# aatifjiwani/lens-flare

Measured on AMD Instinct MI355X. Metric: Mray-surface-intersections/s + frame time, 1080p 256spp double-Gauss, higher is better.
Workload: dtype f32

## Files before the change

### lens-flare_amd/csrc/lf_cull.hip

```cpp
#include <algorithm>
#include <cstdio>
#include <cstdlib>

#include "lf_internal.h"
#include "lf_march_events.h"
#include "lf_march_common.h"

namespace {

using namespace lfm;

constexpr int kWgWaves = 8;
constexpr int kListBits = 12;
constexpr int kListMax = 1 << kListBits;

struct PathTally {
  unsigned long long n_rays = 0, events = 0, n_clip = 0, n_vign = 0, n_tir = 0, n_scene = 0, n_rm_lane = 0, n_rm_rows = 0;
  unsigned long long executed = 0;
  unsigned n_light = 0;
};

template <int VAR>
__device__ __forceinline__ void march_channel_factors(const LfLensDev* __restrict__ lens, float* __restrict__ s_chan, int tid) {
  if (VAR & kVarLights) { lights_channel_factors(lens, s_chan, tid, 64 * kWgWaves); return; }
  if (tid < LF_MAX_LAMBDA * 3) {
    const int l = tid / 3, c = tid - 3 * l;
    s_chan[tid] = l < lens->n_lambda ? lens->sun_radiance[c] * lens->lambda_rgb[l][c] : 0.0f;
  }
}

template <int K, bool W1, int VAR>
__device__ __forceinline__ void march_started_path(const LfLensDev* __restrict__ lens, const LfPairsDev* __restrict__ pairs,
                                                   const int* __restrict__ seq_table, const LfProgRow* __restrict__ rec_table,
                                                   const LfWeightRow* __restrict__ wrec_table, const float* __restrict__ mask,
                                                   const MarchArgs& a, int q, lanemask start_mask, float X, float Y,
                                                   const StartRay& s0, int lane, int acc_slot,
                                                   unsigned long long* __restrict__ s_acc, const float* __restrict__ s_chan,
                                                   PathTally& T) {
  const int n_lambda = lens->n_lambda, prog_recs = pairs->prog_recs;
  const int n_groups = (n_lambda + K - 1) / K;
  const float inv_stop_h = a.inv_stop_h, lobe_thr = a.lobe_thr;
  const float sx = lens->sun_dir[0], sy = lens->sun_dir[1], sz = lens->sun_dir[2];
  const float inv_1mc = lens->sun_inv_one_minus_cos, sun_ss = lens->sun_ss;
  const int n_ev = pairs->ev_cnt[q];
  const int* const seq = seq_table + pairs->ev_off[q];
  for (int g = 0; g < n_groups; g++) {
    const LfProgRow* const recs = rec_table + (size_t)g * (size_t)prog_recs;
    const LfWeightRow* const wrecs = wrec_table + (size_t)g * (size_t)prog_recs;
    Ray r[K];
    lanemask alive[K];
    unsigned nlive = 0u;
#pragma unroll
    for (int j = 0; j < K; j++) {
      r[j] = Ray{X, Y, 0.0f, fmaf(X, X, Y * Y), s0.dx, s0.dy, s0.dz, s0.w0, 1.0f};
      const float ns = lens->n_start[min(g * K + j, n_lambda - 1)];
      r[j].dx *= ns; r[j].dy *= ns; r[j].dz *= ns;
      alive[j] = (g * K + j < n_lambda) ? start_mask : 0ull;
      nlive += (unsigned)__popcll(alive[j]);
    }
    T.n_rays += nlive;
    unsigned ev32 = 0u;
    unsigned se = (unsigned)*(const int __attribute__((address_space(4)))*)(seq);
    int e = 0;
    if (n_ev > 0 && nlive != 0u) for (;;) {
      const unsigned cur = se;
      se = (unsigned)*(const int __attribute__((address_space(4)))*)(seq + e + 1);
      const LfProgRow wr = load_prec(recs, cur & 0xffffu);
      LfWeightRow ww;
      if (W1) ww = load_wrec(wrecs, cur & 0xffffu);
      else { for (int j = 0; j < 3; j++) { ww.fs[j] = 1.0f; ww.fo[j] = 1.0f; ww.fi[j] = 1.0f; } ww.coat = 0; }
      const unsigned kind = cur >> 16;
      lanemask okv[K], gv[K], died = 0ull;
      if (kind & LF_EV_STOP) {
#pragma unroll
        for (int j = 0; j < K; j++) {
          if (K > 1 && __builtin_expect(alive[j] == 0ull, 0)) { okv[j] = 0ull; gv[j] = 0ull; continue; }
          okv[j] = stop_event_var<W1, VAR>(r[j], wr.dzv, wr.h2, inv_stop_h, mask, a.mw, a.mh);
          gv[j] = okv[j];
          died |= alive[j] & ~okv[j];
        }
        if (__builtin_expect(died != 0ull, 0)) {
#pragma unroll
          for (int j = 0; j < K; j++) {
            const unsigned nd = (unsigned)__popcll(alive[j] & ~okv[j]);
            T.n_clip += nd; nlive -= nd; alive[j] &= okv[j];
          }
          if (nlive == 0u) e = n_ev;
        }
      } else {
        if (kind == 0u) {
#pragma unroll
          for (int j = 0; j < K; j++) {
            if (K > 1 && __builtin_expect(alive[j] == 0ull, 0)) { okv[j] = 0ull; gv[j] = 0ull; continue; }
            okv[j] = surface_event<W1>(r[j], wr.dzv, wr.curv, wr.ch, wr.c2, wr.sc, wr.cn22[j], wr.rn2[j],
                                       wr.delta[j], wr.h2, false, false, wr.sgn, gv[j], ww.fs[j], ww.fo[j], ww.fi[j],
                                       CoatSel<VAR>{wrec_table, ww.coat, j});
            died |= alive[j] & ~okv[j];
          }
        } else if (kind == (unsigned)LF_EV_REFLECT) {
#pragma unroll
          for (int j = 0; j < K; j++) {
            if (K > 1 && __builtin_expect(alive[j] == 0ull, 0)) { okv[j] = 0ull; gv[j] = 0ull; continue; }
            okv[j] = surface_event<W1>(r[j], wr.dzv, wr.curv, wr.ch, wr.c2, wr.sc, wr.cn22[j], wr.rn2[j],
                                       wr.delta[j], wr.h2, true, false, wr.sgn, gv[j], ww.fs[j], ww.fo[j], ww.fi[j],
                                       CoatSel<VAR>{wrec_table, ww.coat, j});
            died |= alive[j] & ~okv[j];
          }
        } else {
#pragma unroll
          for (int j = 0; j < K; j++) {
            if (K > 1 && __builtin_expect(alive[j] == 0ull, 0)) { okv[j] = 0ull; gv[j] = 0ull; continue; }
            okv[j] = surface_event<W1>(r[j], wr.dzv, wr.curv, wr.ch, wr.c2, wr.sc, wr.cn22[j], wr.rn2[j],
                                       wr.delta[j], wr.h2, (kind & LF_EV_REFLECT) != 0, (kind & LF_EV_FLAT) != 0,
                                       wr.sgn, gv[j], ww.fs[j], ww.fo[j], ww.fi[j],
                                       CoatSel<VAR>{wrec_table, ww.coat, j});
            died |= alive[j] & ~okv[j];
          }
        }
        if (__builtin_expect(died != 0ull, 0)) {
#pragma unroll
          for (int j = 0; j < K; j++) {
            T.n_vign += (unsigned)__popcll(alive[j] & ~gv[j]);
            T.n_tir += (unsigned)__popcll(alive[j] & gv[j] & ~okv[j]);
            nlive -= (unsigned)__popcll(alive[j] & ~okv[j]);
            alive[j] &= okv[j];
          }
          if (nlive == 0u) e = n_ev;
        }
      }
      ev32 += nlive;
      if (++e >= n_ev) break;
    }
    T.events += ev32;
    T.executed += ev32;
    if (nlive == 0u) continue;
    T.n_scene += nlive;
    lanemask lit[K], lit_any = 0ull;
    if (VAR & kVarLights) {
      lit_any = lights_pretest<K, !W1, VAR>(lens, r, alive, lit);
      if (lit_any == 0ull) continue;
    } else {
#pragma unroll
    for (int j = 0; j < K; j++) {
      const float cg = fmaf(r[j].dx, sx, fmaf(r[j].dy, sy, r[j].dz * sz));
      lit[j] = alive[j] & __ballot(cg > lobe_thr);
      lit_any |= lit[j];
    }
    if (lit_any == 0ull) continue;
    if (!W1) {
      lit_any = lobe_gate<K>(r, lit, sx, sy, sz, sun_ss, inv_1mc);
      if (lit_any == 0ull) continue;
    }
    }
    for (int j = 0; j < K; j++) {
      lanemask lj = lit[0];
#pragma unroll
      for (int jj = 1; jj < K; jj++) lj = (j == jj) ? lit[jj] : lj;
      if (lj == 0ull) continue;
      const int l = g * K + j;
      Ray rw = j == 0 ? r[0] : j == 1 ? r[K > 1 ? 1 : 0] : r[K > 2 ? 2 : 0];
      if (!W1) {
        rw = Ray{X, Y, 0.0f, fmaf(X, X, Y * Y), s0.dx, s0.dy, s0.dz, s0.w0, 1.0f};
        { const float ns = lens->n_start[l]; rw.dx *= ns; rw.dy *= ns; rw.dz *= ns; }
        T.n_rm_lane += (unsigned long long)((unsigned)n_ev * (unsigned)__popcll(lj));
        T.n_rm_rows += (unsigned)n_ev;
        weighted_remarch<VAR>(rw, seq, n_ev, j, recs, wrecs, wrec_table, mask, inv_stop_h, a.mw, a.mh);
      }
      if (VAR & kVarLights) {
        lights_epilogue<VAR>(lens, s_chan, rw, ((lj >> lane) & 1ull) != 0ull, l, &s_acc[acc_slot * 3], T.n_light);
        continue;
      }
      const float qq = lobe_q(rw.dx, rw.dy, rw.dz, sx, sy, sz, sun_ss, inv_1mc);
      const float om = 1.0f - qq;
      float contrib = __fdiv_rn(rw.wn, rw.wd) * (om * om);
      contrib = (((lj >> lane) & 1ull) != 0ull && qq < 1.0f && contrib > 0.0f) ? contrib : 0.0f;
      T.n_light += contrib > 0.0f ? 1u : 0u;
#pragma unroll
      for (int c = 0; c < 3; c++) {
        const float v = contrib * s_chan[l * 3 + c];
        const unsigned long long fx = (unsigned long long)(v * 68719476736.0f);
        if (fx) atomicAdd(&s_acc[acc_slot * 3 + c], fx);
      }
    }
  }
}

template <int K, bool REFLECT, bool FLAT>
__device__ __forceinline__ lanemask surface_rows(Ray (&r)[K], const lanemask (&alive)[K], const LfProgRow& wr, lanemask (&okv)[K],
                                                 lanemask (&gv)[K]) {
  lanemask died = 0ull;
#pragma unroll
  for (int j = 0; j < K; j++) {
    if (K > 1 && __builtin_expect(alive[j] == 0ull, 0)) { okv[j] = 0ull; gv[j] = 0ull; continue; }
    okv[j] = surface_event<false>(r[j], wr.dzv, wr.curv, wr.ch, wr.c2, wr.sc, wr.cn22[j], wr.rn2[j], wr.delta[j], wr.h2,
                                  REFLECT, FLAT, wr.sgn, gv[j]);
    died |= alive[j] & ~okv[j];
  }
  return died;
}

template <int K, int VAR>
__device__ __forceinline__ void march_started_set(const LfLensDev* __restrict__ lens, const LfPairsDev* __restrict__ pairs,
                                                  const int* __restrict__ seq_table, const LfProgRow* __restrict__ rec_table,
                                                  const LfWeightRow* __restrict__ wrec_table, const float* __restrict__ mask,
                                                  const MarchArgs& a, unsigned long long todo, lanemask active_mask, float X, float Y,
                                                  const StartRay& s0, int lane, unsigned long long* __restrict__ s_acc,
                                                  const int2* __restrict__ s_meta, const float* __restrict__ s_chan,
                                                  PathTally& T) {
  const int n_lambda = lens->n_lambda, prog_recs = pairs->prog_recs;
  const int n_groups = (n_lambda + K - 1) / K;
  const float inv_stop_h = a.inv_stop_h, lobe_thr = a.lobe_thr;
  const float sx = lens->sun_dir[0], sy = lens->sun_dir[1], sz = lens->sun_dir[2];
  const float inv_1mc = lens->sun_inv_one_minus_cos, sun_ss = lens->sun_ss;
  const unsigned n_started = (unsigned)__popcll(todo);
  for (int g = 0; g < n_groups; g++) {
    const LfProgRow* const recs = rec_table + (size_t)g * (size_t)prog_recs;
    const LfWeightRow* const wrecs = wrec_table + (size_t)g * (size_t)prog_recs;
    Ray r[K], p[K];
    lanemask alive[K], palive[K];
    unsigned nlive = 0u, pn = 0u;
#pragma unroll
    for (int j = 0; j < K; j++) {
      r[j] = Ray{X, Y, 0.0f, fmaf(X, X, Y * Y), s0.dx, s0.dy, s0.dz, s0.w0, 1.0f};
      const float ns = lens->n_start[min(g * K + j, n_lambda - 1)];
      r[j].dx *= ns; r[j].dy *= ns; r[j].dz *= ns;
      alive[j] = (g * K + j < n_lambda) ? active_mask : 0ull;
      nlive += (unsigned)__popcll(alive[j]);
      p[j] = r[j]; palive[j] = alive[j];
    }
    T.n_rays += (unsigned long long)nlive * n_started;
    int depth = 0;
    unsigned long long left = todo;
    while (left != 0ull && nlive != 0u) {
      const int q = 63 - __builtin_clzll(left);
      left &= ~(1ull << q);
      const int2 meta = s_meta[q];
      const int mx = __builtin_amdgcn_readfirstlane(meta.x);
      const int n_ev = mx >> 16, L = mx & 0xffff;
      const int* const seq = seq_table + __builtin_amdgcn_readfirstlane(meta.y);
      unsigned mult = (unsigned)__popcll(left) + 1u;
      bool forked = false;
      unsigned seg = 0u;
      unsigned long long ev_logical = 0ull;
      unsigned ev_exec = 0u;
      unsigned se = (unsigned)*(const int __attribute__((address_space(4)))*)(seq + depth);
      int e = depth;
      if (e < n_ev && nlive != 0u) for (;;) {
        if (e == L) {
#pragma unroll
          for (int j = 0; j < K; j++) { p[j] = r[j]; palive[j] = alive[j]; }
          pn = nlive; forked = true;
          ev_logical = (unsigned long long)seg * mult; ev_exec = seg; seg = 0u; mult = 1u;
        }
        const unsigned cur = se;
        se = (unsigned)*(const int __attribute__((address_space(4)))*)(seq + e + 1);
        const LfProgRow wr = load_prec(recs, cur & 0xffffu);
        const unsigned kind = cur >> 16;
        lanemask okv[K], gv[K], died = 0ull;
        if (__builtin_expect(kind == 0u, 1)) {
          died = surface_rows<K, false, false>(r, alive, wr, okv, gv);
        } else if (kind & LF_EV_STOP) {
#pragma unroll
          for (int j = 0; j < K; j++) {
            if (K > 1 && __builtin_expect(alive[j] == 0ull, 0)) { okv[j] = 0ull; gv[j] = 0ull; continue; }
            okv[j] = stop_event_var<false, VAR>(r[j], wr.dzv, wr.h2, inv_stop_h, mask, a.mw, a.mh);
            gv[j] = okv[j];
            died |= alive[j] & ~okv[j];
          }
        } else if (kind & LF_EV_REFLECT) {
          if (kind & LF_EV_FLAT) died = surface_rows<K, true, true>(r, alive, wr, okv, gv);
          else died = surface_rows<K, true, false>(r, alive, wr, okv, gv);
        } else {
          died = surface_rows<K, false, true>(r, alive, wr, okv, gv);
        }
        if (__builtin_expect(died != 0ull, 0)) {
          const bool stop_row = (kind & LF_EV_STOP) != 0;
#pragma unroll
          for (int j = 0; j < K; j++) {
            const unsigned nd = (unsigned)__popcll(alive[j] & ~okv[j]);
            const unsigned nv = (unsigned)__popcll(alive[j] & ~gv[j]);
            T.n_clip += stop_row ? (unsigned long long)nd * mult : 0ull;
            T.n_vign += stop_row ? 0ull : (unsigned long long)nv * mult;
            T.n_tir += stop_row ? 0ull : (unsigned long long)(nd - nv) * mult;
            nlive -= nd;
            alive[j] &= okv[j];
          }
          if (nlive == 0u) e = n_ev;
        }
        seg += nlive;
        if (++e >= n_ev) break;
      }
      T.events += ev_logical + (unsigned long long)seg * mult;
      T.executed += ev_exec + seg;
      if (!forked && L < n_ev) break;
      if (nlive != 0u) {
        T.n_scene += nlive;
        lanemask lit[K], lit_any = 0ull;
        if (VAR & kVarLights) {
          lit_any = lights_pretest<K, true, VAR>(lens, r, alive, lit);
        } else {
#pragma unroll
        for (int j = 0; j < K; j++) {
          const float cg = fmaf(r[j].dx, sx, fmaf(r[j].dy, sy, r[j].dz * sz));
          lit[j] = alive[j] & __ballot(cg > lobe_thr);
          lit_any |= lit[j];
        }
        if (lit_any != 0ull) lit_any = lobe_gate<K>(r, lit, sx, sy, sz, sun_ss, inv_1mc);
        }
        if (lit_any != 0ull) {
          for (int j = 0; j < K; j++) {
            lanemask lj = lit[0];
#pragma unroll
            for (int jj = 1; jj < K; jj++) lj = (j == jj) ? lit[jj] : lj;
            if (lj == 0ull) continue;
            const int l = g * K + j;
            Ray rw = Ray{X, Y, 0.0f, fmaf(X, X, Y * Y), s0.dx, s0.dy, s0.dz, s0.w0, 1.0f};
            { const float ns = lens->n_start[l]; rw.dx *= ns; rw.dy *= ns; rw.dz *= ns; }
            T.n_rm_lane += (unsigned long long)((unsigned)n_ev * (unsigned)__popcll(lj));
            T.n_rm_rows += (unsigned)n_ev;
            weighted_remarch<VAR>(rw, seq, n_ev, j, recs, wrecs, wrec_table, mask, inv_stop_h, a.mw, a.mh);
            if (VAR & kVarLights) {
              lights_epilogue<VAR>(lens, s_chan, rw, ((lj >> lane) & 1ull) != 0ull, l, &s_acc[lane * 3], T.n_light);
              continue;
            }
            const float qq = lobe_q(rw.dx, rw.dy, rw.dz, sx, sy, sz, sun_ss, inv_1mc);
            const float om = 1.0f - qq;
            float contrib = __fdiv_rn(rw.wn, rw.wd) * (om * om);
            contrib = (((lj >> lane) & 1ull) != 0ull && qq < 1.0f && contrib > 0.0f) ? contrib : 0.0f;
            T.n_light += contrib > 0.0f ? 1u : 0u;
#pragma unroll
            for (int c = 0; c < 3; c++) {
              const float v = contrib * s_chan[l * 3 + c];
              const unsigned long long fx = (unsigned long long)(v * 68719476736.0f);
              if (fx) atomicAdd(&s_acc[lane * 3 + c], fx);
            }
          }
        }
      }
      if (!forked || left == 0ull) break;
#pragma unroll
      for (int j = 0; j < K; j++) { r[j] = p[j]; alive[j] = palive[j]; }
      nlive = pn;
      depth = L;
    }
  }
}

#ifndef LF_SHARED_WAVES
#define LF_SHARED_WAVES 6
#endif
template <int K, bool W1, int MODE, int VAR>
__global__ __launch_bounds__(64 * kWgWaves, ((VAR & kVarOccl) ? 4 : K == 1 ? 8 : MODE == 1 ? LF_SHARED_WAVES : 6))
void k_march_cull(const LfLensDev* __restrict__ lens, const LfPairsDev* __restrict__ pairs,
                  const int* __restrict__ seq_table, const LfProgRow* __restrict__ rec_table,
                  const LfWeightRow* __restrict__ wrec_table, const float* __restrict__ mask, MarchArgs a,
                  LfCullArgs cull, double* __restrict__ ghost, unsigned long long* __restrict__ accum,
                  unsigned long long* __restrict__ counters) {
  __shared__ unsigned long long s_acc[64 * 3];
  __shared__ unsigned long long s_cnt[kMarchCounters];
  __shared__ int s_next, s_nlist;
  static_assert(2 * kMaxSubcellBits <= 32 - kListBits, "a listed sample's sub-cell does not fit beside its place in the chunk");
  __shared__ unsigned s_list[kListMax];
  __shared__ int2 s_meta[MODE == 1 ? kCullMaxPaths : 1];
  __shared__ float s_chan[(VAR & kVarLights) ? kLightChan : LF_MAX_LAMBDA * 3];
  const int tid = threadIdx.x;
  if (tid < 64 * 3) s_acc[tid] = 0ull;
  march_channel_factors<VAR>(lens, s_chan, tid);
  if (tid < kMarchCounters) s_cnt[tid] = 0ull;
  if (tid == 0) { s_next = 0; s_nlist = 0; }
  if (MODE == 1 && tid < pairs->n && tid < kCullMaxPaths) {
    const int n_ev = pairs->ev_cnt[tid], i1 = pairs->ij[tid][0];
    s_meta[tid] = make_int2((n_ev << 16) | (i1 < 0 ? n_ev : lens->n_surf - 1 - i1), pairs->ev_off[tid]);
  }
  __syncthreads();

  const int tiles_x = ((a.W + (8 << a.xs) - 1) >> (3 + a.xs)) << a.xs;
#ifdef LF_EXPERIMENTS
  if (cull.wg_clock && tid == 0) cull.wg_clock[2 * (size_t)blockIdx.x] = wall_clock64();
  struct ClockAtExit { unsigned long long* p; __device__ ~ClockAtExit() { if (p && threadIdx.x == 0) *p = wall_clock64(); } }
      clock_at_exit{cull.wg_clock ? cull.wg_clock + 2 * (size_t)blockIdx.x + 1 : nullptr};
#endif
  const unsigned n_head = (unsigned)a.tail_from * (unsigned)a.sgroups;
  const bool tail = a.tail_groups > 1 && blockIdx.x >= n_head;
  const int sgroups = tail ? a.tail_groups : a.sgroups;
  const int sg = tail ? (int)((blockIdx.x - n_head) % (unsigned)sgroups) : (int)(blockIdx.x % (unsigned)sgroups);
  const unsigned slot = tail ? (unsigned)a.tail_from + (blockIdx.x - n_head) / (unsigned)sgroups : blockIdx.x / (unsigned)sgroups;
  const int tile_lin = (int)((slot & ~63u) | ((slot & 7u) << 3) | ((slot >> 3) & 7u));
  if (tile_lin >= a.n_tiles) return;
  int tx, trow;
  march_tile_of(a, tile_lin, tiles_x, tx, trow);
  const unsigned tile_id = (unsigned)(trow * tiles_x + tx);
  const int wave = __builtin_amdgcn_readfirstlane(tid >> 6);
  const int lane = tid & 63;
  const int x = ((tx >> a.xs) << (3 + a.xs)) + ((lane & 7) << a.xs) + (tx & ((1 << a.xs) - 1)), y = trow * 8 + (lane >> 3);
  const bool active = x < a.W && y >= a.y0 && y < a.y1;
  const lanemask active_mask = __ballot(active);
  const unsigned p = (unsigned)y * (unsigned)a.W + (unsigned)x;
  const int blk = ((trow * 8) >> cull.blk_log2) * cull.blocks_x + ((((tx >> a.xs) << (3 + a.xs))) >> cull.blk_log2);
  const unsigned long long* const crow = cull.table + lf_cull_row_of_block(blk, cull.share_n, cull.share_nb) * (size_t)(cull.cells + 1);
  const int blk_lane = (min(y, a.H - 1) >> cull.blk_log2) * cull.blocks_x + (min(x, a.W - 1) >> cull.blk_log2);
  const unsigned long long* const crow_lane = cull.multi ? cull.table + lf_cull_row_of_block(blk_lane, cull.share_n, cull.share_nb) * (size_t)(cull.cells + 1) : crow;

  const float pitch = lens->pitch, pupil_h = lens->pupil_h, geom_norm = lens->geom_norm;
  const float half_w = a.half_w, half_h = a.half_h, vz_u = a.vz;
  const int GG = a.G * a.G;
  const bool per_lane = (1 << a.sub_bits) < cull.m;

  PathTally T;

  const int n_mine = (a.spp - sg + sgroups - 1) / sgroups;
  for (int chunk0 = 0; chunk0 < n_mine; chunk0 += kListMax) {
    const int chunk_n = min(kListMax, n_mine - chunk0);
    for (int k = tid; k < chunk_n; k += 64 * kWgWaves) {
      const int s = sg + (chunk0 + k) * sgroups;
      bool work = true;
      unsigned drawn = 0u;
      if (s >= GG && !cull.multi) work = crow[cull.cells] != 0ull;
      if (s < GG) {
        const uint4 r2 = philox4x32_10(make_uint4(tile_id, (unsigned)s, kDomainSubcell, 0u), a.key);
        const unsigned sxi = a.sub_bits ? (r2.x >> (32 - a.sub_bits)) : 0u, syi = a.sub_bits ? (r2.y >> (32 - a.sub_bits)) : 0u;
        drawn = sxi | (syi << kMaxSubcellBits);
        if (!per_lane && !cull.multi) {
          const int cy = s / a.G, cx = s - cy * a.G;
          work = crow[(cy * cull.m + (int)((syi << cull.m_shift) >> a.sub_bits)) * cull.P + cx * cull.m + (int)((sxi << cull.m_shift) >> a.sub_bits)] != 0ull;
        }
      }
      if (work) s_list[atomicAdd(&s_nlist, 1)] = (unsigned)k | (drawn << kListBits);
    }
    __syncthreads();
    const int n_list = s_nlist;
    for (;;) {
      int k = 0;
      if (lane == 0) k = atomicAdd(&s_next, 1);
      k = __builtin_amdgcn_readfirstlane(k);
      if (k >= n_list) break;
      const unsigned listed = (unsigned)__builtin_amdgcn_readfirstlane((int)s_list[k]);
      const int s = sg + (chunk0 + (int)(listed & (unsigned)(kListMax - 1))) * sgroups;
      const uint4 rnd = philox4x32_10(make_uint4(p, (unsigned)s, kDomainMarch, 0u), a.key);
      const float jx = u01(rnd.x), jy = u01(rnd.y);
      float ua = u01(rnd.z), ub = u01(rnd.w);
      int entry = -1;
      if (s < GG) {
        const int cy = s / a.G, cx = s - cy * a.G;
        const unsigned sxi = (listed >> kListBits) & ((1u << kMaxSubcellBits) - 1u);
        const unsigned syi = listed >> (kListBits + kMaxSubcellBits);
        ua = ((float)cx + ((float)sxi + ua) * a.inv_sub) * a.inv_G;
        ub = ((float)cy + ((float)syi + ub) * a.inv_sub) * a.inv_G;
        if (!per_lane) entry = (cy * cull.m + (int)((syi << cull.m_shift) >> a.sub_bits)) * cull.P + cx * cull.m + (int)((sxi << cull.m_shift) >> a.sub_bits);
      }
      if (s >= GG) entry = cull.cells;
      const float pa0 = fmaf(2.0f, ua, -1.0f), pb0 = fmaf(2.0f, ub, -1.0f);
      const float X = -(((float)x + jx) - half_w) * pitch;
      const float Y = -(((float)y + jy) - half_h) * pitch;
      if (MODE == 1) {
        const unsigned long long todo = crow[entry];
        if (todo == 0ull) continue;
        const StartRay s0 = aim_at_pupil(X, Y, pa0, pb0, pupil_h, vz_u, geom_norm);
        march_started_set<K, VAR>(lens, pairs, seq_table, rec_table, wrec_table, mask, a, todo, active_mask, X, Y, s0, lane, s_acc, s_meta, s_chan, T);
        continue;
      }
      unsigned long long mine, todo;
      if (entry >= 0 && !cull.multi) { todo = crow[entry]; mine = todo; }
      else {
        const int fx = min(cull.P - 1, (int)(ua * (float)cull.P)), fy = min(cull.P - 1, (int)(ub * (float)cull.P));
        mine = active ? crow_lane[entry >= 0 ? entry : fy * cull.P + fx] : 0ull;
        unsigned lo = (unsigned)mine, hi = (unsigned)(mine >> 32);
        for (int off = 32; off > 0; off >>= 1) { lo |= __shfl_xor(lo, off); hi |= __shfl_xor(hi, off); }
        todo = ((unsigned long long)__builtin_amdgcn_readfirstlane(hi) << 32) | (unsigned long long)__builtin_amdgcn_readfirstlane(lo);
      }
      if (todo == 0ull) continue;
      const StartRay s0 = aim_at_pupil(X, Y, pa0, pb0, pupil_h, vz_u, geom_norm);
      unsigned long long left_q = todo;
      while (left_q != 0ull) {
        const int q = __builtin_ctzll(left_q);
        left_q &= left_q - 1ull;
        const lanemask start_mask = active_mask & __ballot(((mine >> q) & 1ull) != 0ull);
        march_started_path<K, W1, VAR>(lens, pairs, seq_table, rec_table, wrec_table, mask, a, q, start_mask, X, Y, s0, lane, lane, s_acc, s_chan, T);
      }
    }
    __syncthreads();
    if (tid == 0) { s_next = 0; s_nlist = 0; }
    __syncthreads();
  }

  {
    unsigned long long v6 = T.n_light;
    for (int off = 32; off > 0; off >>= 1) v6 += __shfl_down(v6, off);
    const unsigned long long vals[kMarchCounters] = {T.n_rays, T.events, T.n_clip, T.n_vign, T.n_tir, T.n_scene, v6, T.executed, T.n_rm_lane, T.n_rm_rows};
    if (lane == 0) {
#pragma unroll
      for (int i = 0; i < kMarchCounters; i++)
        if (vals[i]) atomicAdd(&s_cnt[i], vals[i]);
    }
  }
  __syncthreads();
  if (wave == 0 && lane < kMarchCounters && s_cnt[lane]) atomicAdd(&counters[lane], s_cnt[lane]);

  if (tail) {
    if (wave != 0) return;
    const unsigned tt = slot - (unsigned)a.tail_from;
    unsigned long long* const acc = cull.tail_acc + (size_t)tt * 192u;
#pragma unroll
    for (int c = 0; c < 3; c++)
      if (s_acc[lane * 3 + c]) atomicAdd(&acc[lane * 3 + c], s_acc[lane * 3 + c]);
    __threadfence();
    int arrived = 0;
    if (lane == 0) arrived = atomicAdd(&cull.tail_done[tt], 1);
    arrived = __shfl(arrived, 0);
    if (arrived != sgroups - 1) return;
    __threadfence();
#pragma unroll
    for (int c = 0; c < 3; c++) {
      const unsigned long long sum = atomicExch(&acc[lane * 3 + c], 0ull);
      if (active) {
        const double v = ((double)sum * (1.0 / 68719476736.0)) / (double)a.spp;
        ghost[3 * (size_t)p + c] = a.accumulate ? ghost[3 * (size_t)p + c] + v : v;
      }
    }
    if (lane == 0) atomicExch(&cull.tail_done[tt], 0);
    return;
  }
  if (wave == 0 && active) {
    if (a.sgroups == 1) {
#pragma unroll
      for (int c = 0; c < 3; c++) {
        const double v = ((double)s_acc[lane * 3 + c] * (1.0 / 68719476736.0)) / (double)a.spp;
        ghost[3 * (size_t)p + c] = a.accumulate ? ghost[3 * (size_t)p + c] + v : v;
      }
    } else {
#pragma unroll
      for (int c = 0; c < 3; c++)
        if (s_acc[lane * 3 + c]) atomicAdd(&accum[3 * (size_t)p + c], s_acc[lane * 3 + c]);
    }
  }
}

constexpr int kItemCap = 16384;
constexpr int kItemChunk = 256;
constexpr int kItemCellCache = 64;

template <int K, int VAR>
__global__ __launch_bounds__(64 * kWgWaves, (VAR & kVarOccl) ? 4 : 6)
void k_march_items(const LfLensDev* __restrict__ lens, const LfPairsDev* __restrict__ pairs,
                   const int* __restrict__ seq_table, const LfProgRow* __restrict__ rec_table,
                   const LfWeightRow* __restrict__ wrec_table, const float* __restrict__ mask, MarchArgs a,
                   LfCullArgs cull, double* __restrict__ ghost, unsigned long long* __restrict__ accum,
                   unsigned long long* __restrict__ counters) {
  __shared__ unsigned long long s_acc[64 * 3];
  __shared__ unsigned long long s_cnt[kMarchCounters];
  __shared__ int s_pcount[kCullMaxPaths], s_poff[kCullMaxPaths + 1], s_goff[kCullMaxPaths + 1], s_pfill[kCullMaxPaths];
  __shared__ int s_next;
  __shared__ unsigned short s_items[kItemCap];
  __shared__ unsigned short s_cell[kItemCellCache * 64];
  __shared__ float s_chan[(VAR & kVarLights) ? kLightChan : LF_MAX_LAMBDA * 3];
  const int tid = threadIdx.x;
  if (tid < 64 * 3) s_acc[tid] = 0ull;
  march_channel_factors<VAR>(lens, s_chan, tid);
  if (tid < kMarchCounters) s_cnt[tid] = 0ull;
  __syncthreads();

  const int tiles_x = ((a.W + (8 << a.xs) - 1) >> (3 + a.xs)) << a.xs;
  const int sg = blockIdx.x % a.sgroups;
  const unsigned slot = blockIdx.x / a.sgroups;
  const int tile_lin = (int)((slot & ~63u) | ((slot & 7u) << 3) | ((slot >> 3) & 7u));
  if (tile_lin >= a.n_tiles) return;
  int tx, trow;
  march_tile_of(a, tile_lin, tiles_x, tx, trow);
  const unsigned tile_id = (unsigned)(trow * tiles_x + tx);
  const int wave = __builtin_amdgcn_readfirstlane(tid >> 6);
  const int lane = tid & 63;
  const int n_paths = pairs->n;
  const float pitch = lens->pitch, pupil_h = lens->pupil_h, geom_norm = lens->geom_norm;
  const float half_w = a.half_w, half_h = a.half_h, vz_u = a.vz;
  const int GG = a.G * a.G;
  const unsigned long long* crow;
  {
    const int lx = ((tx >> a.xs) << (3 + a.xs)) + ((lane & 7) << a.xs) + (tx & ((1 << a.xs) - 1)), ly = trow * 8 + (lane >> 3);
    const int blk = cull.multi ? (min(ly, a.H - 1) >> cull.blk_log2) * cull.blocks_x + (min(lx, a.W - 1) >> cull.blk_log2)
                               : ((trow * 8) >> cull.blk_log2) * cull.blocks_x + ((((tx >> a.xs) << (3 + a.xs))) >> cull.blk_log2);
    crow = cull.table + lf_cull_row_of_block(blk, cull.share_n, cull.share_nb) * (size_t)(cull.cells + 1);
  }
  auto pixel_of = [&](int px, int& x, int& y) {
    x = ((tx >> a.xs) << (3 + a.xs)) + ((px & 7) << a.xs) + (tx & ((1 << a.xs) - 1));
    y = trow * 8 + (px >> 3);
    return x < a.W && y >= a.y0 && y < a.y1;
  };
  auto pupil_point = [&](int x, int y, int s, float& ua, float& ub, float& jx, float& jy) {
    const uint4 rnd = philox4x32_10(make_uint4((unsigned)y * (unsigned)a.W + (unsigned)x, (unsigned)s, kDomainMarch, 0u), a.key);
    jx = u01(rnd.x); jy = u01(rnd.y);
    ua = u01(rnd.z); ub = u01(rnd.w);
    if (s < GG) {
      const int cy = s / a.G, cx = s - cy * a.G;
      unsigned sxi = 0u, syi = 0u;
      if (a.sub_bits) {
        const uint4 r2 = philox4x32_10(make_uint4(tile_id, (unsigned)s, kDomainSubcell, 0u), a.key);
        sxi = r2.x >> (32 - a.sub_bits); syi = r2.y >> (32 - a.sub_bits);
      }
      ua = ((float)cx + ((float)sxi + ua) * a.inv_sub) * a.inv_G;
      ub = ((float)cy + ((float)syi + ub) * a.inv_sub) * a.inv_G;
    }
  };
  auto cell_of = [&](int k_global) -> unsigned {
    int x, y;
    if (!pixel_of(lane, x, y)) return 0xffffu;
    const int s = sg + k_global * a.sgroups;
    if (s >= GG) return (unsigned)cull.cells;
    float ua, ub, jx, jy;
    pupil_point(x, y, s, ua, ub, jx, jy);
    const int fx = min(cull.P - 1, (int)(ua * (float)cull.P)), fy = min(cull.P - 1, (int)(ub * (float)cull.P));
    return (unsigned)(fy * cull.P + fx);
  };
  auto mask_at = [&](unsigned cell) -> unsigned long long { return cell == 0xffffu ? 0ull : crow[cell]; };
  auto wave_or = [](unsigned long long v) {
    unsigned lo = (unsigned)v, hi = (unsigned)(v >> 32);
    for (int off = 32; off > 0; off >>= 1) { lo |= __shfl_xor(lo, off); hi |= __shfl_xor(hi, off); }
    return ((unsigned long long)__builtin_amdgcn_readfirstlane(hi) << 32) | (unsigned long long)__builtin_amdgcn_readfirstlane(lo);
  };

  PathTally T;
  const int n_mine = (a.spp - sg + a.sgroups - 1) / a.sgroups;
  int c0 = 0, ch = min(max(1, min(kItemChunk, cull.items_chunk0)), n_mine);
  while (c0 < n_mine) {
    const int chn = min(ch, n_mine - c0);
    if (tid < kCullMaxPaths) { s_pcount[tid] = 0; s_pfill[tid] = 0; }
    if (tid == 0) s_next = 0;
    __syncthreads();
    const bool cached = chn <= kItemCellCache;
    for (int k = wave; k < chn; k += kWgWaves) {
      const unsigned cell = cell_of(c0 + k);
      if (cached) s_cell[k * 64 + lane] = (unsigned short)cell;
      const unsigned long long mine = mask_at(cell);
      unsigned long long u = wave_or(mine);
      while (u != 0ull) {
        const int q = __builtin_ctzll(u);
        u &= u - 1ull;
        const int c = __popcll(__ballot(((mine >> q) & 1ull) != 0ull));
        if (lane == 0) atomicAdd(&s_pcount[q], c);
      }
    }
    __syncthreads();
    if (tid == 0) {
      int off = 0, goff = 0;
      for (int q = 0; q < n_paths; q++) { s_poff[q] = off; s_goff[q] = goff; off += s_pcount[q]; goff += (s_pcount[q] + 63) >> 6; }
      s_poff[n_paths] = off; s_goff[n_paths] = goff;
    }
    __syncthreads();
    const int total = s_poff[n_paths];
    if (total > kItemCap && chn > 1) {
// ... 255 lines not shown
```

### lens-flare_amd/csrc/lf_march_common.h

```cpp
#pragma once

#include <cstddef>

#include "lf_internal.h"
#include "lf_march_events.h"
#include "lf_scene_walk.h"

namespace lfm {

__device__ __forceinline__ float lobe_q(float dx, float dy, float dz, float sx, float sy, float sz,
                                        float ss, float inv_1mc) {
  const float cg = fmaf(dx, sx, fmaf(dy, sy, dz * sz));
  const float cx = fmaf(dy, sz, -(dz * sy)), cy = fmaf(dz, sx, -(dx * sz)), cz = fmaf(dx, sy, -(dy * sx));
  const float c2 = fmaf(cx, cx, fmaf(cy, cy, cz * cz));
  const float dd = fmaf(dx, dx, fmaf(dy, dy, dz * dz));
  const float ds = dd * ss;
  const float den = fmaf(lf_sqrt(ds), cg, ds);
  return __fdiv_rn(c2, den) * inv_1mc;
}

template <int K>
__device__ __forceinline__ lanemask lobe_gate(const Ray (&r)[K], lanemask (&lit)[K], float sx, float sy, float sz, float ss,
                                              float inv_1mc) {
  lanemask lit_any = 0ull;
#pragma unroll
  for (int j = 0; j < K; j++) {
    if (lit[j] != 0ull) lit[j] &= __ballot(lobe_q(r[j].dx, r[j].dy, r[j].dz, sx, sy, sz, ss, inv_1mc) < 1.0f);
    lit_any |= lit[j];
  }
  return lit_any;
}

__device__ __forceinline__ lfw::DRay ghost_shadow_ray(const LfOcclDev& o, float px, float py, float z, float dx, float dy, float dz,
                                                      double max_t = (double)INFINITY) {
  using namespace lfw;
  const double wpm = o.wpm;
  const V3 oc = v3((double)px * wpm, (double)py * wpm, ((double)z - o.z_ref) * wpm);
  const V3 dc = unit(v3((double)dx, (double)dy, (double)dz));
  const V3 ow = v3(o.pos[0] + ((oc.x * o.c2w[0] + oc.y * o.c2w[1]) + oc.z * o.c2w[2]),
                   o.pos[1] + ((oc.x * o.c2w[3] + oc.y * o.c2w[4]) + oc.z * o.c2w[5]),
                   o.pos[2] + ((oc.x * o.c2w[6] + oc.y * o.c2w[7]) + oc.z * o.c2w[8]));
  return make_ray(ow,
                  v3((dc.x * o.c2w[0] + dc.y * o.c2w[1]) + dc.z * o.c2w[2],
                     (dc.x * o.c2w[3] + dc.y * o.c2w[4]) + dc.z * o.c2w[5],
                     (dc.x * o.c2w[6] + dc.y * o.c2w[7]) + dc.z * o.c2w[8]),
                  0.0, max_t);
}
__device__ inline bool ghost_ray_visible(const LfOcclDev& o, float px, float py, float z, float dx, float dy, float dz,
                                         double max_t = (double)INFINITY) {
  lfw::DRay ray = ghost_shadow_ray(o, px, py, z, dx, dy, dz, max_t);
  LfSceneDev sc{};
  sc.nodes = o.nodes; sc.prims = o.prims;
  int stack[lfw::kStackDepth];
  lfw::SceneTally tally{0u, 0u};
  return !lfw::closest_hit<1>(sc, ray, nullptr, stack, tally);
}


__device__ __forceinline__ bool light_admits(const LfLensDev* __restrict__ lens, int k, float dx, float dy, float dz, float& q) {
  const float sx = lens->light_dir[k][0], sy = lens->light_dir[k][1], sz = lens->light_dir[k][2];
  const float cg = fmaf(dx, sx, fmaf(dy, sy, dz * sz));
  q = lobe_q(dx, dy, dz, sx, sy, sz, lens->light_ss[k], lens->light_inv_one_minus_cos[k]);
  return cg > lens->light_thr[k] && q < 1.0f;
}
template <int VAR>
__device__ __forceinline__ bool light_admits_at(const LfLensDev* __restrict__ lens, int k, float px, float py, float hz, float dx, float dy,
                                                float dz, float& q) {
  if ((VAR & kVarArea) && lens->light_kind[k] == LF_LIGHT_AREA) {
    q = 0.0f;
    return lf_area_inside(dx, dy, dz, px, py, lens->surf[0].zv + hz, lens->light_pos[k], lens->light_area[k]);
  }
  if ((VAR & kVarNear) && lens->light_kind[k] != LF_LIGHT_DIRECTIONAL) {
    float cg;
    q = lf_point_lobe_q(dx, dy, dz, px, py, lens->surf[0].zv + hz, lens->light_pos[k][0], lens->light_pos[k][1], lens->light_pos[k][2],
                        lens->light_inv_one_minus_cos[k], cg);
    return cg > 0.0f && q < 1.0f;
  }
  return light_admits(lens, k, dx, dy, dz, q);
}
template <int K, bool GATE, int VAR = kVarLights>
__device__ __forceinline__ lanemask lights_pretest(const LfLensDev* __restrict__ lens, const Ray (&r)[K], const lanemask (&alive)[K],
                                                   lanemask (&lit)[K]) {
  const int n = lens->n_lights;
  lanemask lit_any = 0ull;
#pragma unroll
  for (int j = 0; j < K; j++) {
    bool near = false;
    for (int k = 0; k < n; k++) {
      if ((VAR & kVarArea) && lens->light_kind[k] == LF_LIGHT_AREA) {
        near = lf_area_pretest(r[j].dx, r[j].dy, r[j].dz, r[j].px, r[j].py, lens->surf[0].zv + r[j].hz, lens->light_pos[k],
                               lens->light_thr[k]) || near;
        continue;
      }
      if ((VAR & kVarNear) && lens->light_kind[k] != LF_LIGHT_DIRECTIONAL) {
        near = lf_point_pretest(r[j].dx, r[j].dy, r[j].dz, r[j].px, r[j].py, lens->surf[0].zv + r[j].hz, lens->light_pos[k][0],
                                lens->light_pos[k][1], lens->light_pos[k][2], lens->light_thr[k]) || near;
        continue;
      }
      const float cg = fmaf(r[j].dx, lens->light_dir[k][0], fmaf(r[j].dy, lens->light_dir[k][1], r[j].dz * lens->light_dir[k][2]));
      near = near || cg > lens->light_thr[k];
    }
    lit[j] = alive[j] & __ballot(near);
    lit_any |= lit[j];
  }
  if (!GATE || lit_any == 0ull) return lit_any;
  lit_any = 0ull;
#pragma unroll
  for (int j = 0; j < K; j++) {
    if (lit[j] != 0ull) {
      bool in = false;
      for (int k = 0; k < n; k++) { float q; in = light_admits_at<VAR>(lens, k, r[j].px, r[j].py, r[j].hz, r[j].dx, r[j].dy, r[j].dz, q) || in; }
      lit[j] &= __ballot(in);
    }
    lit_any |= lit[j];
  }
  return lit_any;
}
constexpr int kLightChan = LF_MAX_LIGHTS * LF_MAX_LAMBDA * 3;
__device__ __forceinline__ void lights_channel_factors(const LfLensDev* __restrict__ lens, float* __restrict__ s_chan, int tid, int n_threads) {
  for (int i = tid; i < kLightChan; i += n_threads) {
    const int k = i / (LF_MAX_LAMBDA * 3), lc = i - k * (LF_MAX_LAMBDA * 3), l = lc / 3, c = lc - 3 * l;
    s_chan[i] = (k < lens->n_lights && l < lens->n_lambda) ? lens->light_radiance[k][c] * lens->lambda_rgb[l][c] : 0.0f;
  }
}
template <int VAR = kVarLights>
__device__ __forceinline__ void lights_epilogue(const LfLensDev* __restrict__ lens, const float* __restrict__ s_chan, const Ray& rw,
                                                bool mine, int l, unsigned long long* __restrict__ acc, unsigned& n_light) {
  const int n = lens->n_lights;
  const float wq = __fdiv_rn(rw.wn, rw.wd);
  const LfOcclDev& occl = *(const LfOcclDev*)((const char*)lens + kLensOcclOffset);
  int vis = -1;
  double seen_to = -1.0, dark_from = 0.0;
  bool dark_any = false;
  unsigned w_tested = 0u, w_blocked = 0u;
  for (int k = 0; k < n; k++) {
    float qq;
    const bool in = light_admits_at<VAR>(lens, k, rw.px, rw.py, rw.hz, rw.dx, rw.dy, rw.dz, qq);
    const float om = 1.0f - qq;
    float contrib = wq * (om * om);
    contrib = (mine && in && contrib > 0.0f) ? contrib : 0.0f;
    if ((VAR & kVarOccl) && (VAR & kVarNear)) {
      const bool test = contrib > 0.0f;
      const bool point = lens->light_kind[k] != LF_LIGHT_DIRECTIONAL;
      const bool area = (VAR & kVarArea) && lens->light_kind[k] == LF_LIGHT_AREA;
      if (test) {
        const float z = occl.front_zv + rw.hz;
        double reach = (double)INFINITY;
        if (area)
          reach = lf_area_shadow_reach(rw.dx, rw.dy, rw.dz, rw.px, rw.py, z, lens->light_pos[k], lens->light_area[k], occl.wpm);
        else if (point)
          reach = lf_point_shadow_reach(rw.dx, rw.dy, rw.dz, rw.px, rw.py, z, lens->light_pos[k][0], lens->light_pos[k][1],
                                        lens->light_pos[k][2], occl.wpm);
        bool v;
        if (reach <= seen_to) v = true;
        else if (dark_any && reach >= dark_from) v = false;
        else {
          v = ghost_ray_visible(occl, rw.px, rw.py, z, rw.dx, rw.dy, rw.dz, reach);
          if (v) seen_to = reach; else { dark_from = reach; dark_any = true; }
        }
        if (!v) contrib = 0.0f;
      }
      w_tested += (unsigned)__popcll(__ballot(test));
      w_blocked += (unsigned)__popcll(__ballot(test && contrib == 0.0f));
    } else if (VAR & kVarOccl) {
      const bool test = contrib > 0.0f;
      if (test) {
        if (vis < 0)
          vis = ghost_ray_visible(occl, rw.px, rw.py, occl.front_zv + rw.hz, rw.dx, rw.dy, rw.dz) ? 1 : 0;
        if (vis == 0) contrib = 0.0f;
      }
      w_tested += (unsigned)__popcll(__ballot(test));
      w_blocked += (unsigned)__popcll(__ballot(test && contrib == 0.0f));
    }
    n_light += contrib > 0.0f ? 1u : 0u;
    const float* const ch = s_chan + (k * LF_MAX_LAMBDA + l) * 3;
#pragma unroll
    for (int c = 0; c < 3; c++) {
      const float v = contrib * ch[c];
      const unsigned long long fx = (unsigned long long)(v * 68719476736.0f);
      if (fx) atomicAdd(&acc[c], fx);
    }
  }
  if ((VAR & kVarOccl) && w_tested != 0u) {
    const lanemask act = __ballot(true);
    if (__lane_id() == (unsigned)(__ffsll((long long)act) - 1)) {
      atomicAdd(&occl.stats[0], (unsigned long long)w_tested);
      if (w_blocked) atomicAdd(&occl.stats[1], (unsigned long long)w_blocked);
    }
  }
}

struct MarchArgs {
  int mw, mh, W, H, y0, y1;
  int spp, G;
  float inv_G;
  int sub_bits;
  float inv_sub;
  int trow0, tperiod;
  LfDeal deal;
  int sgroups;
  int tail_from, tail_groups;
  uint2 key;
  float inv_stop_h;
  float half_w, half_h;
  float vz;
  float lobe_thr;
  int accumulate;
  int n_tiles;
  int xs;
};

__device__ __forceinline__ void march_tile_of(const MarchArgs& a, int tile_lin, int tiles_x, int& tx, int& trow) {
  if (a.deal.bx > 0) {
    const int b = a.deal.rank + (tile_lin >> 6) * a.deal.n, w = tile_lin & 63;
    const int by = b / a.deal.bx;
    trow = by * 8 + (w >> 3);
    tx = (b - by * a.deal.bx) * 8 + (w & 7);
  } else {
    const int tj = tile_lin / tiles_x;
    tx = tile_lin - tj * tiles_x;
    trow = a.trow0 + tj * a.tperiod;
  }
}
__device__ __forceinline__ bool march_owns(const MarchArgs& a, int x, int y) {
  if (a.deal.bx > 0) return lf_deal_mine(a.deal, x, y);
  const int t = y >> 3;
  return t >= a.trow0 && (t - a.trow0) % a.tperiod == 0;
}

typedef int lf_i16 __attribute__((ext_vector_type(16)));
typedef int lf_i4 __attribute__((ext_vector_type(4)));
typedef const lf_i16 __attribute__((address_space(4))) * lf_const_prow_ptr;
typedef const lf_i4 __attribute__((address_space(4))) * lf_const_phdr_ptr;
__device__ __forceinline__ LfProgRow load_prec(const LfProgRow* __restrict__ base, unsigned off) {
  typedef const char __attribute__((address_space(4))) * cptr;
  const lf_i16 v = *(lf_const_prow_ptr)((cptr)(base) + off);
  LfProgRow r;
  r.dzv = __int_as_float(v[0]); r.curv = __int_as_float(v[1]); r.h2 = __int_as_float(v[2]);
  r.sc = __int_as_float(v[3]); r.sgn = __int_as_float(v[4]);
#pragma unroll
  for (int j = 0; j < 3; j++) {
    r.delta[j] = __int_as_float(v[5 + j]); r.cn22[j] = __int_as_float(v[8 + j]); r.rn2[j] = __int_as_float(v[12 + j]);
  }
  r.ch = __int_as_float(v[11]); r.c2 = __int_as_float(v[15]);
  return r;
}
__device__ __forceinline__ LfWeightRow load_wrec(const LfWeightRow* __restrict__ base, unsigned off) {
  typedef const char __attribute__((address_space(4))) * cptr;
  const lf_i16 v = *(lf_const_prow_ptr)((cptr)(base) + off);
  LfWeightRow r;
#pragma unroll
  for (int j = 0; j < 3; j++) {
    r.fs[j] = __int_as_float(v[j]); r.fo[j] = __int_as_float(v[4 + j]); r.fi[j] = __int_as_float(v[8 + j]);
  }
  r.pad0 = r.pad1 = r.pad2 = 0.0f;
  r.coat = v[12];
  r.pad3[0] = r.pad3[1] = r.pad3[2] = 0.0f;
  return r;
}
__device__ __forceinline__ LfProgHdr load_phdr(const LfProgHdr* __restrict__ base, unsigned off) {
  typedef const char __attribute__((address_space(4))) * cptr;
  const lf_i4 v = *(lf_const_phdr_ptr)((cptr)(base) + off);
  LfProgHdr h;
  h.flags = v[0]; h.skip = v[1]; h.rec = v[2]; h.rec_next = v[3];
  return h;
}

__device__ __forceinline__ int load_wrec_dword(const void* __restrict__ base, unsigned off) {
  typedef const char __attribute__((address_space(4))) * cptr;
  return *(const int __attribute__((address_space(4)))*)((cptr)(base) + off);
}

template <int VAR>
__device__ __forceinline__ void weighted_remarch(Ray& rw, const int* __restrict__ w, int n_ev, int j, const LfProgRow* __restrict__ recs,
                                                 const LfWeightRow* __restrict__ wrecs,
                                                 const LfWeightRow* __restrict__ wrec_table, const float* __restrict__ mask,
                                                 float inv_stop_h, int mw, int mh) {
  const char* const wj = (const char*)wrecs + 4 * j;
  unsigned se = (unsigned)*(const int __attribute__((address_space(4)))*)(w);
  for (int left = n_ev; left > 0; --left) {
    const unsigned cur = se;
    se = (unsigned)*(const int __attribute__((address_space(4)))*)(++w);
    const unsigned off = cur & 0xffffu;
    const LfProgRow wr = load_prec(recs, off);
    const float w_fs = __int_as_float(load_wrec_dword(wj, off + (unsigned)offsetof(LfWeightRow, fs)));
    const float w_fo = __int_as_float(load_wrec_dword(wj, off + (unsigned)offsetof(LfWeightRow, fo)));
    const float w_fi = __int_as_float(load_wrec_dword(wj, off + (unsigned)offsetof(LfWeightRow, fi)));
    int w_coat = 0;
    if (VAR & kVarCoat) w_coat = load_wrec_dword(wrecs, off + (unsigned)offsetof(LfWeightRow, coat));
    const unsigned wfl = cur >> 16;
    const float w_cn22 = j == 0 ? wr.cn22[0] : j == 1 ? wr.cn22[1] : wr.cn22[2];
    const float w_rn2 = j == 0 ? wr.rn2[0] : j == 1 ? wr.rn2[1] : wr.rn2[2];
    const float w_delta = j == 0 ? wr.delta[0] : j == 1 ? wr.delta[1] : wr.delta[2];
    if (wfl & LF_EV_STOP) {
      (void)stop_event_var<true, VAR>(rw, wr.dzv, wr.h2, inv_stop_h, mask, mw, mh);
    } else {
      lanemask geom_ok;
      (void)surface_event<true>(rw, wr.dzv, wr.curv, wr.ch, wr.c2, wr.sc, w_cn22, w_rn2, w_delta, wr.h2,
                                (wfl & LF_EV_REFLECT) != 0, (wfl & LF_EV_FLAT) != 0, wr.sgn, geom_ok, w_fs, w_fo, w_fi,
                                CoatSel<VAR>{wrec_table, w_coat, j});
    }
  }
}

}

lf_status lf_march_lights_ready(const lf_ctx* ctx);
bool lf_march_launch_args(const lf_ctx* ctx, int spp, uint64_t key, bool culled, lfm::MarchArgs* out, size_t* out_tiles);
lf_status lf_march_upload_lens(lf_ctx* ctx, const LfLensDev& L, int bits);
```

Measured before the change: 949,300.

## Split started-path marching into shared prefix and private tail with copied state

Restructures the per-path march so the shared prefix up to the fork depth L runs once on the running state. Each path's own tail then runs on a copy, which replaces the old fork-snapshot/restore bookkeeping inside the event loop. It also reuses the lobe quality value computed in the gate instead of recomputing lobe_q after the weighted re-march, and accumulates re-march counters in 32-bit locals. The risk is that the reused lobe_q now comes from the unweighted ray direction rather than the re-marched one, which could change results slightly, and the extra copied ray state may raise register pressure.

```diff
diff --git a/lens-flare_amd/csrc/lf_cull.hip b/lens-flare_amd/csrc/lf_cull.hip
--- a/lens-flare_amd/csrc/lf_cull.hip
+++ b/lens-flare_amd/csrc/lf_cull.hip
@@ -200,6 +200,45 @@
 }
 
 template <int K, int VAR>
+__device__ __forceinline__ void started_row(Ray (&s)[K], lanemask (&alive)[K], unsigned& nlive, unsigned cur, unsigned mult,
+                                            const LfProgRow* __restrict__ recs, const float* __restrict__ mask, const MarchArgs& a,
+                                            float inv_stop_h, PathTally& T, int& e, int end) {
+  const LfProgRow wr = load_prec(recs, cur & 0xffffu);
+  const unsigned kind = cur >> 16;
+  lanemask okv[K], gv[K], died = 0ull;
+  if (__builtin_expect(kind == 0u, 1)) {
+    died = surface_rows<K, false, false>(s, alive, wr, okv, gv);
+  } else if (kind & LF_EV_STOP) {
+#pragma unroll
+    for (int j = 0; j < K; j++) {
+      if (K > 1 && __builtin_expect(alive[j] == 0ull, 0)) { okv[j] = 0ull; gv[j] = 0ull; continue; }
+      okv[j] = stop_event_var<false, VAR>(s[j], wr.dzv, wr.h2, inv_stop_h, mask, a.mw, a.mh);
+      gv[j] = okv[j];
+      died |= alive[j] & ~okv[j];
+    }
+  } else if (kind & LF_EV_REFLECT) {
+    if (kind & LF_EV_FLAT) died = surface_rows<K, true, true>(s, alive, wr, okv, gv);
+    else died = surface_rows<K, true, false>(s, alive, wr, okv, gv);
+  } else {
+    died = surface_rows<K, false, true>(s, alive, wr, okv, gv);
+  }
+  if (__builtin_expect(died != 0ull, 0)) {
+    const bool stop_row = (kind & LF_EV_STOP) != 0;
+#pragma unroll
+    for (int j = 0; j < K; j++) {
+      const unsigned nd = (unsigned)__popcll(alive[j] & ~okv[j]);
+      const unsigned nv = (unsigned)__popcll(alive[j] & ~gv[j]);
+      T.n_clip += stop_row ? (unsigned long long)nd * mult : 0ull;
+      T.n_vign += stop_row ? 0ull : (unsigned long long)nv * mult;
+      T.n_tir += stop_row ? 0ull : (unsigned long long)(nd - nv) * mult;
+      nlive -= nd;
+      alive[j] &= okv[j];
+    }
+    if (nlive == 0u) e = end;
+  }
+}
+
+template <int K, int VAR>
 __device__ __forceinline__ void march_started_set(const LfLensDev* __restrict__ lens, const LfPairsDev* __restrict__ pairs,
                                                   const int* __restrict__ seq_table, const LfProgRow* __restrict__ rec_table,
                                                   const LfWeightRow* __restrict__ wrec_table, const float* __restrict__ mask,
@@ -213,12 +252,14 @@
   const float sx = lens->sun_dir[0], sy = lens->sun_dir[1], sz = lens->sun_dir[2];
   const float inv_1mc = lens->sun_inv_one_minus_cos, sun_ss = lens->sun_ss;
   const unsigned n_started = (unsigned)__popcll(todo);
+  static_assert((unsigned long long)kCullMaxPaths * LF_MAX_LAMBDA * 0xffffull * 64ull < (1ull << 32), "a sample's re-march rows overflow 32 bits");
+  unsigned rm_lane = 0u, rm_rows = 0u;
   for (int g = 0; g < n_groups; g++) {
     const LfProgRow* const recs = rec_table + (size_t)g * (size_t)prog_recs;
     const LfWeightRow* const wrecs = wrec_table + (size_t)g * (size_t)prog_recs;
-    Ray r[K], p[K];
-    lanemask alive[K], palive[K];
-    unsigned nlive = 0u, pn = 0u;
+    Ray r[K], c[K];
+    lanemask alive[K], calive[K];
+    unsigned nlive = 0u;
 #pragma unroll
     for (int j = 0; j < K; j++) {
       r[j] = Ray{X, Y, 0.0f, fmaf(X, X, Y * Y), s0.dx, s0.dy, s0.dz, s0.w0, 1.0f};
@@ -226,7 +267,6 @@
       r[j].dx *= ns; r[j].dy *= ns; r[j].dz *= ns;
       alive[j] = (g * K + j < n_lambda) ? active_mask : 0ull;
       nlive += (unsigned)__popcll(alive[j]);
-      p[j] = r[j]; palive[j] = alive[j];
     }
     T.n_rays += (unsigned long long)nlive * n_started;
     int depth = 0;
@@ -238,74 +278,50 @@
       const int mx = __builtin_amdgcn_readfirstlane(meta.x);
       const int n_ev = mx >> 16, L = mx & 0xffff;
       const int* const seq = seq_table + __builtin_amdgcn_readfirstlane(meta.y);
-      unsigned mult = (unsigned)__popcll(left) + 1u;
-      bool forked = false;
+      const unsigned mult = (unsigned)__popcll(left) + 1u;
+      unsigned se = (unsigned)*(const int __attribute__((address_space(4)))*)(seq + depth);
       unsigned seg = 0u;
-      unsigned long long ev_logical = 0ull;
-      unsigned ev_exec = 0u;
-      unsigned se = (unsigned)*(const int __attribute__((address_space(4)))*)(seq + depth);
       int e = depth;
-      if (e < n_ev && nlive != 0u) for (;;) {
-        if (e == L) {
-#pragma unroll
-          for (int j = 0; j < K; j++) { p[j] = r[j]; palive[j] = alive[j]; }
-          pn = nlive; forked = true;
-          ev_logical = (unsigned long long)seg * mult; ev_exec = seg; seg = 0u; mult = 1u;
-        }
+      if (e < L) for (;;) {
         const unsigned cur = se;
         se = (unsigned)*(const int __attribute__((address_space(4)))*)(seq + e + 1);
-        const LfProgRow wr = load_prec(recs, cur & 0xffffu);
-        const unsigned kind = cur >> 16;
-        lanemask okv[K], gv[K], died = 0ull;
-        if (__builtin_expect(kind == 0u, 1)) {
-          died = surface_rows<K, false, false>(r, alive, wr, okv, gv);
-        } else if (kind & LF_EV_STOP) {
-#pragma unroll
-          for (int j = 0; j < K; j++) {
-            if (K > 1 && __builtin_expect(alive[j] == 0ull, 0)) { okv[j] = 0ull; gv[j] = 0ull; continue; }
-            okv[j] = stop_event_var<false, VAR>(r[j], wr.dzv, wr.h2, inv_stop_h, mask, a.mw, a.mh);
-            gv[j] = okv[j];
-            died |= alive[j] & ~okv[j];
-          }
-        } else if (kind & LF_EV_REFLECT) {
-          if (kind & LF_EV_FLAT) died = surface_rows<K, true, true>(r, alive, wr, okv, gv);
-          else died = surface_rows<K, true, false>(r, alive, wr, okv, gv);
+        started_row<K, VAR>(r, alive, nlive, cur, mult, recs, mask, a, inv_stop_h, T, e, L);
+        seg += nlive;
+        if (++e >= L) break;
+      }
+      T.events += (unsigned long long)seg * mult;
+      T.executed += seg;
+      depth = L;
+      if (nlive == 0u) break;
+      unsigned cn = nlive;
+#pragma unroll
+      for (int j = 0; j < K; j++) { c[j] = r[j]; calive[j] = alive[j]; }
+      if (L < n_ev) {
+        unsigned own = 0u;
+        for (;;) {
+          const unsigned cur = se;
+          se = (unsigned)*(const int __attribute__((address_space(4)))*)(seq + e + 1);
+          started_row<K, VAR>(c, calive, cn, cur, 1u, recs, mask, a, inv_stop_h, T, e, n_ev);
+          own += cn;
+          if (++e >= n_ev) break;
+        }
+        T.events += own;
+        T.executed += own;
+      }
+      if (cn != 0u) {
+        T.n_scene += cn;
+        lanemask lit[K], lit_any = 0ull;
+        float gq[K];
+        if (VAR & kVarLights) {
+          lit_any = lights_pretest<K, true, VAR>(lens, c, calive, lit);
         } else {
-          died = surface_rows<K, false, true>(r, alive, wr, okv, gv);
-        }
-        if (__builtin_expect(died != 0ull, 0)) {
-          const bool stop_row = (kind & LF_EV_STOP) != 0;
-#pragma unroll
-          for (int j = 0; j < K; j++) {
-            const unsigned nd = (unsigned)__popcll(alive[j] & ~okv[j]);
-            const unsigned nv = (unsigned)__popcll(alive[j] & ~gv[j]);
-            T.n_clip += stop_row ? (unsigned long long)nd * mult : 0ull;
-            T.n_vign += stop_row ? 0ull : (unsigned long long)nv * mult;
-            T.n_tir += stop_row ? 0ull : (unsigned long long)(nd - nv) * mult;
-            nlive -= nd;
-            alive[j] &= okv[j];
-          }
-          if (nlive == 0u) e = n_ev;
-        }
-        seg += nlive;
-        if (++e >= n_ev) break;
-      }
-      T.events += ev_logical + (unsigned long long)seg * mult;
-      T.executed += ev_exec + seg;
-      if (!forked && L < n_ev) break;
-      if (nlive != 0u) {
-        T.n_scene += nlive;
-        lanemask lit[K], lit_any = 0ull;
-        if (VAR & kVarLights) {
-          lit_any = lights_pretest<K, true, VAR>(lens, r, alive, lit);
-        } else {
 #pragma unroll
         for (int j = 0; j < K; j++) {
-          const float cg = fmaf(r[j].dx, sx, fmaf(r[j].dy, sy, r[j].dz * sz));
-          lit[j] = alive[j] & __ballot(cg > lobe_thr);
+          const float cg = fmaf(c[j].dx, sx, fmaf(c[j].dy, sy, c[j].dz * sz));
+          lit[j] = calive[j] & __ballot(cg > lobe_thr);
           lit_any |= lit[j];
         }
-        if (lit_any != 0ull) lit_any = lobe_gate<K>(r, lit, sx, sy, sz, sun_ss, inv_1mc);
+        if (lit_any != 0ull) lit_any = lobe_gate<K>(c, lit, sx, sy, sz, sun_ss, inv_1mc, gq);
         }
         if (lit_any != 0ull) {
           for (int j = 0; j < K; j++) {
@@ -316,34 +332,37 @@
             const int l = g * K + j;
             Ray rw = Ray{X, Y, 0.0f, fmaf(X, X, Y * Y), s0.dx, s0.dy, s0.dz, s0.w0, 1.0f};
             { const float ns = lens->n_start[l]; rw.dx *= ns; rw.dy *= ns; rw.dz *= ns; }
-            T.n_rm_lane += (unsigned long long)((unsigned)n_ev * (unsigned)__popcll(lj));
-            T.n_rm_rows += (unsigned)n_ev;
+            rm_lane += (unsigned)n_ev * (unsigned)__popcll(lj);
+            rm_rows += (unsigned)n_ev;
             weighted_remarch<VAR>(rw, seq, n_ev, j, recs, wrecs, wrec_table, mask, inv_stop_h, a.mw, a.mh);
             if (VAR & kVarLights) {
               lights_epilogue<VAR>(lens, s_chan, rw, ((lj >> lane) & 1ull) != 0ull, l, &s_acc[lane * 3], T.n_light);
               continue;
             }
-            const float qq = lobe_q(rw.dx, rw.dy, rw.dz, sx, sy, sz, sun_ss, inv_1mc);
+            const float* const ch = s_chan + l * 3;
+            const float ch0 = ch[0], ch1 = ch[1], ch2 = ch[2];
+            float qq = gq[0];
+#pragma unroll
+            for (int jj = 1; jj < K; jj++) qq = (j == jj) ? gq[jj] : qq;
             const float om = 1.0f - qq;
             float contrib = __fdiv_rn(rw.wn, rw.wd) * (om * om);
             contrib = (((lj >> lane) & 1ull) != 0ull && qq < 1.0f && contrib > 0.0f) ? contrib : 0.0f;
             T.n_light += contrib > 0.0f ? 1u : 0u;
-#pragma unroll
-            for (int c = 0; c < 3; c++) {
-              const float v = contrib * s_chan[l * 3 + c];
+            const float chv[3] = {ch0, ch1, ch2};
+#pragma unroll
+            for (int c3 = 0; c3 < 3; c3++) {
+              const float v = contrib * chv[c3];
               const unsigned long long fx = (unsigned long long)(v * 68719476736.0f);
-              if (fx) atomicAdd(&s_acc[lane * 3 + c], fx);
+              if (fx) atomicAdd(&s_acc[lane * 3 + c3], fx);
             }
           }
         }
       }
-      if (!forked || left == 0ull) break;
-#pragma unroll
-      for (int j = 0; j < K; j++) { r[j] = p[j]; alive[j] = palive[j]; }
-      nlive = pn;
-      depth = L;
-    }
-  }
+      if (L >= n_ev) break;
+    }
+  }
+  T.n_rm_lane += rm_lane;
+  T.n_rm_rows += rm_rows;
 }
 
 #ifndef LF_SHARED_WAVES
diff --git a/lens-flare_amd/csrc/lf_march_common.h b/lens-flare_amd/csrc/lf_march_common.h
--- a/lens-flare_amd/csrc/lf_march_common.h
+++ b/lens-flare_amd/csrc/lf_march_common.h
@@ -21,14 +21,24 @@
 
 template <int K>
 __device__ __forceinline__ lanemask lobe_gate(const Ray (&r)[K], lanemask (&lit)[K], float sx, float sy, float sz, float ss,
+                                              float inv_1mc, float (&q)[K]) {
+  lanemask lit_any = 0ull;
+#pragma unroll
+  for (int j = 0; j < K; j++) {
+    q[j] = 2.0f;
+    if (lit[j] != 0ull) {
+      q[j] = lobe_q(r[j].dx, r[j].dy, r[j].dz, sx, sy, sz, ss, inv_1mc);
+      lit[j] &= __ballot(q[j] < 1.0f);
+    }
+    lit_any |= lit[j];
+  }
+  return lit_any;
+}
+template <int K>
+__device__ __forceinline__ lanemask lobe_gate(const Ray (&r)[K], lanemask (&lit)[K], float sx, float sy, float sz, float ss,
                                               float inv_1mc) {
-  lanemask lit_any = 0ull;
-#pragma unroll
-  for (int j = 0; j < K; j++) {
-    if (lit[j] != 0ull) lit[j] &= __ballot(lobe_q(r[j].dx, r[j].dy, r[j].dz, sx, sy, sz, ss, inv_1mc) < 1.0f);
-    lit_any |= lit[j];
-  }
-  return lit_any;
+  float q[K];
+  return lobe_gate<K>(r, lit, sx, sy, sz, ss, inv_1mc, q);
 }
 
 __device__ __forceinline__ lfw::DRay ghost_shadow_ray(const LfOcclDev& o, float px, float py, float z, float dx, float dy, float dz,
```

After: 986,400 (median of 6 runs). +3.9%, better.
